# RchalYang/torchrl

Hardware: AMD Instinct MI355X
Metric: env_steps_per_sec_ppo_2048env_halfcheetah_shape (higher is better)
Workload: dtype f32

## Files before the change

torchrl_amd/csrc/k_rollout.hip:

```cpp
#include <algorithm>
#include "trl_common.h"
#include "trl_mlp.h"
#include "trl_head.h"
#include "trl_philox.h"

#define RO_THREADS 256
#define RO_ENVS 16
#ifdef TRL_EXP_CLK
#define CLK_DECL long long clk_prev = clock64(); float clk_acc[8] = {0, 0, 0, 0, 0, 0, 0, 0};
#define CLK(ph) { const long long c_ = clock64(); clk_acc[ph] += (float)(c_ - clk_prev); clk_prev = c_; }
#else
#define CLK_DECL
#define CLK(ph)
#endif
#define RO_NB 16

struct RolloutDev {
  const float *pf_params, *vf_params, *env_A, *env_B;
  float reward_scale; int horizon; int64_t env_seed_base;
  float* cur_obs; int32_t *t_env, *cur_step, *episode_idx; float* ep_return;
  const float* noise; int64_t noise_step0;
  float *obs, *next_obs, *acts, *values, *rewards, *terminals, *time_limits, *old_logp;
  int rows, top, N, n_steps, max_episode_frames; float discount;
  double* epoch_reward; int32_t* ep_count; float* ep_log; int ep_cap; int step0;
  int tanh_action, deterministic, store;
  double* norm_state; float* policy_obs; double* norm_ws; float norm_clip; int norm_update, norm_partial_reset;
  double* clear_hdr;
  float* boot;
  uint32_t* pub_dst; const uint32_t* pub_src; int64_t pub_words;
  const uint32_t* noise_flag; uint32_t noise_stamp;
  int D, A;
  int n_ro_wg; const f32x4* stg_src; unsigned long long* stg_dst; int64_t stg_n4;
  const uint32_t* stg_ready; uint32_t stg_job; uint32_t* stg_state; uint32_t* stg_ack;
  int64_t cat_seed, cat_env0;
};
#define RO_STAGERS 16

template <int CTRL> __device__ __forceinline__ double ro_dpp_f64(double v) {
  const unsigned long long u = __builtin_bit_cast(unsigned long long, v);
  const unsigned lo = (unsigned)__builtin_amdgcn_update_dpp(0, (int)(unsigned)(u & 0xFFFFFFFFull), CTRL, 0xF, 0xF, false);
  const unsigned hi = (unsigned)__builtin_amdgcn_update_dpp(0, (int)(unsigned)(u >> 32), CTRL, 0xF, 0xF, false);
  return __builtin_bit_cast(double, ((unsigned long long)hi << 32) | lo);
}
__device__ __forceinline__ double ro_row_sum16(double v) {
  v += ro_dpp_f64<0x128>(v);
  v += ro_dpp_f64<0x124>(v);
  v += ro_dpp_f64<0x122>(v);
  v += ro_dpp_f64<0x121>(v);
  return v;
}
#define NORM_SLOT 40

template <int D, int H, int A, int HC_ = 8> struct RoShape {
  static_assert(H == 64 && D > 16 && D <= 32 && A <= 8, "instantiated for 16 < D <= 32, H == 64, A <= 8");
  static_assert(HC_ == 8 || HC_ == 16, "the head exchange carries half or all of the 16-row head tile");
  static constexpr int HC = HC_;
  static constexpr int O_B1 = 0, O_B2 = H, O_B3 = 2 * H, O_LS = O_B3 + HC, O_H1 = O_LS + 8, O_HP = O_H1 + H * TL,
                       O_EPS = O_HP + 4 * HC * 16, LDS_FLOATS = O_EPS + RO_NB * 8 * 16;
};

__device__ __forceinline__ void stage_block(const f32x4* __restrict__ src, unsigned long long* __restrict__ dst, int64_t n4,
                                            int wg, int wgs, int threads, uint32_t* __restrict__ state, uint32_t stamp,
                                            uint32_t* __restrict__ host_ack) {
  const int64_t stride = (int64_t)wgs * threads;
  for (int64_t e = (int64_t)wg * threads + threadIdx.x; e < n4; e += 4 * stride) {
    f32x4 v[4];
#pragma unroll
    for (int q = 0; q < 4; ++q) if (e + q * stride < n4) v[q] = src[e + q * stride];
#pragma unroll
    for (int q = 0; q < 4; ++q)
      if (e + q * stride < n4) {
        const unsigned long long lo = ((unsigned long long)__float_as_uint(v[q][1]) << 32) | __float_as_uint(v[q][0]);
        const unsigned long long hi = ((unsigned long long)__float_as_uint(v[q][3]) << 32) | __float_as_uint(v[q][2]);
        __hip_atomic_store(dst + 2 * (e + q * stride), lo, __ATOMIC_RELAXED, __HIP_MEMORY_SCOPE_AGENT);
        __hip_atomic_store(dst + 2 * (e + q * stride) + 1, hi, __ATOMIC_RELAXED, __HIP_MEMORY_SCOPE_AGENT);
      }
  }
  asm volatile("s_waitcnt vmcnt(0)" ::: "memory");
  __syncthreads();
  if (threadIdx.x == 0) {
    const unsigned before = __hip_atomic_fetch_add(state + 1, 1u, __ATOMIC_RELAXED, __HIP_MEMORY_SCOPE_AGENT);
    if (before == (unsigned)wgs - 1) {
      __hip_atomic_store(state + 1, 0u, __ATOMIC_RELAXED, __HIP_MEMORY_SCOPE_AGENT);
      __hip_atomic_store(state, stamp, __ATOMIC_RELAXED, __HIP_MEMORY_SCOPE_AGENT);
      if (host_ack) __hip_atomic_store(host_ack, stamp, __ATOMIC_RELAXED, __HIP_MEMORY_SCOPE_SYSTEM);
    }
  }
}

template <int D, int H, int A, int ACT, bool NORM, bool RT = false, int HEAD = HEAD_GAUSS>
__global__ __launch_bounds__(RO_THREADS, 1) void rollout_kernel(RolloutDev a) {
  using S = RoShape<D, H, A, HEAD == HEAD_SD ? 16 : 8>;
  constexpr bool WIDE = D > 17, CAT = HEAD == HEAD_CAT, SD = HEAD == HEAD_SD;
  static_assert(!CAT || RT, "the categorical head exists as a runtime-dims instantiation only");
  static_assert(!SD || (RT && !NORM), "the state-dependent-std head exists as a runtime-dims instantiation only");
  static_assert(!WIDE || RT, "the wide tile exists as a runtime-dims instantiation only");
  static_assert(!(RT && NORM), "the cooperative (normalised) rollout is instantiated for the benchmark shape");
  const int Dr = RT ? a.D : D, Ar = RT ? a.A : A;
  const int HW = SD ? 2 * Ar : Ar;
  const int F_W1 = 0, F_B1 = H * Dr, F_W2 = F_B1 + H, F_B2 = F_W2 + H * H, F_W3 = F_B2 + H, F_B3 = F_W3 + HW * H,
            F_LS = F_B3 + HW;
  __shared__ __attribute__((aligned(16))) float lds[S::LDS_FLOATS];
  if (!NORM && (int)blockIdx.x >= a.n_ro_wg) {
    __shared__ int s_go;
    if (threadIdx.x == 0) {
      const unsigned long long t0 = wall_clock64();
      int go = 1;
      while (__hip_atomic_load(a.stg_ready, __ATOMIC_RELAXED, __HIP_MEMORY_SCOPE_SYSTEM) != a.stg_job) {
        __builtin_amdgcn_s_sleep(64);
        if (wall_clock64() - t0 > 3000ull) { go = 0; break; }
      }
      s_go = go;
    }
    __syncthreads();
    if (s_go)
      stage_block(a.stg_src, a.stg_dst, a.stg_n4, (int)blockIdx.x - a.n_ro_wg, (int)gridDim.x - a.n_ro_wg, RO_THREADS,
                  a.stg_state, a.stg_job, a.stg_ack);
    return;
  }
  const int tid = threadIdx.x, lane = tid & 63;
  const int mo = __builtin_amdgcn_readfirstlane(tid >> 6);
  const int j = lane & 15, g = lane >> 4, i = j;
  const int n = blockIdx.x * RO_ENVS + j;
  const bool valid = n < a.N;
  const float* gp = a.pf_params;
  const bool has_lo = g < Ar, has_hi = 4 + g < Ar;
  const int o_lo = has_lo ? g : 0, o_hi = has_hi ? 4 + g : 0;
  if (blockIdx.x == 0 && tid == 0 && a.clear_hdr) { a.clear_hdr[0] = 0.0; a.clear_hdr[1] = 0.0; }
  if (a.noise_flag && tid == 0) {
    unsigned spins = 0;
    while (__hip_atomic_load(a.noise_flag, __ATOMIC_RELAXED, __HIP_MEMORY_SCOPE_AGENT) != a.noise_stamp) {
      __builtin_amdgcn_s_sleep(32);
      if (++spins > (1u << 24)) {
        if (blockIdx.x == 0 && a.epoch_reward) a.epoch_reward[0] = __builtin_nan("");
        break;
      }
    }
    if (spins) __threadfence();
  }

  for (int e = tid; e < H; e += RO_THREADS) { lds[S::O_B1 + e] = gp[F_B1 + e]; lds[S::O_B2 + e] = gp[F_B2 + e]; }
  if constexpr (SD) {
    if (tid < 16) lds[S::O_B3 + tid] = tid < HW ? gp[F_B3 + (tid < HW ? tid : 0)] : 0.0f;
    if (tid < 8) lds[S::O_LS + tid] = 0.0f;
  } else if (tid < 8) {
    lds[S::O_B3 + tid] = tid < Ar ? gp[F_B3 + (tid < Ar ? tid : 0)] : 0.0f;
    lds[S::O_LS + tid] = (!CAT && tid < Ar) ? gp[F_LS + (tid < Ar ? tid : 0)] : 0.0f;
  }
  bool fv[4], fv2[4];
#pragma unroll
  for (int q = 0; q < 4; ++q) { fv[q] = 4 * g + q < Dr; fv2[q] = WIDE && 16 + 4 * g + q < Dr; }
  const bool f16 = !WIDE && 16 + g < Dr;
  const bool row_f = i < Dr, row_f2 = WIDE && 16 + i < Dr;
  constexpr int XK = WIDE ? 8 : 5, EK = XK + 2;
  float w1r[XK], w2r[4][4], w3a[4], we0[EK], w16[EK], we1[WIDE ? EK : 1];
  {
    const int row = 16 * mo + i;
#pragma unroll
    for (int r = 0; r < 4; ++r) w1r[r] = fv[r] ? gp[F_W1 + row * Dr + (fv[r] ? 4 * g + r : 0)] : 0.0f;
    if constexpr (WIDE) {
#pragma unroll
      for (int r = 0; r < 4; ++r) w1r[4 + r] = fv2[r] ? gp[F_W1 + row * Dr + (fv2[r] ? 16 + 4 * g + r : 0)] : 0.0f;
    } else {
      w1r[4] = f16 ? gp[F_W1 + row * Dr + (f16 ? 16 + g : 0)] : 0.0f;
    }
#pragma unroll
    for (int sl = 0; sl < 4; ++sl)
#pragma unroll
      for (int r = 0; r < 4; ++r) w2r[sl][r] = gp[F_W2 + row * H + 16 * sl + 4 * g + r];
#pragma unroll
    for (int r = 0; r < 4; ++r) w3a[r] = (i < HW) ? gp[F_W3 + (i < HW ? i : 0) * H + 16 * mo + 4 * g + r] : 0.0f;
    static_assert(WIDE || D == 17, "the narrow env step keeps exactly one feature outside the 16-row MFMA tile");
    const bool has16 = !WIDE && Dr > 16;
#pragma unroll
    for (int q = 0; q < EK; ++q) {
      const float* mat = q < XK ? a.env_A : a.env_B;
      int k; bool kin;
      if (q < 4) { k = 4 * g + q; kin = k < Dr; }
      else if (q < XK) { k = WIDE ? 16 + 4 * g + (q - 4) : 16 + g; kin = k < Dr; }
      else { k = (q == XK) ? g : 4 + g; kin = k < Ar; }
      const int kc = kin ? k : 0;
      we0[q] = (kin && row_f) ? mat[kc * Dr + (row_f ? i : 0)] : 0.0f;
      w16[q] = (kin && has16) ? mat[kc * Dr + (has16 ? 16 : 0)] : 0.0f;
      if constexpr (WIDE) we1[q] = (kin && row_f2) ? mat[kc * Dr + (row_f2 ? 16 + i : 0)] : 0.0f;
    }
  }
  __syncthreads();

  float* S_H1 = lds + S::O_H1;
  float* headp = lds + S::O_HP;
  float* S_EPS = lds + S::O_EPS;
  const float* b1s = lds + S::O_B1 + 16 * mo + 4 * g;
  const float* b2s = lds + S::O_B2 + 16 * mo + 4 * g;

  float ls_lo = fminf(fmaxf(lds[S::O_LS + o_lo], -20.0f), 2.0f), ls_hi = fminf(fmaxf(lds[S::O_LS + o_hi], -20.0f), 2.0f);
  float std_lo = __expf(ls_lo), std_hi = __expf(ls_hi);
  float iv_lo = __expf(-2.0f * ls_lo), iv_hi = __expf(-2.0f * ls_hi);
  const float b3_lo = lds[S::O_B3 + o_lo], b3_hi = lds[S::O_B3 + o_hi];

  float xb[XK];
#pragma unroll
  for (int r = 0; r < 4; ++r) xb[r] = (valid && fv[r]) ? a.cur_obs[(size_t)n * Dr + (fv[r] ? 4 * g + r : 0)] : 0.0f;
  if constexpr (WIDE) {
#pragma unroll
    for (int r = 0; r < 4; ++r) xb[4 + r] = (valid && fv2[r]) ? a.cur_obs[(size_t)n * Dr + (fv2[r] ? 16 + 4 * g + r : 0)] : 0.0f;
  } else {
    xb[4] = (valid && f16) ? a.cur_obs[(size_t)n * Dr + (f16 ? 16 + g : 0)] : 0.0f;
  }
  float xp[XK];
  __shared__ double s_mean[NORM ? D : 1], s_var[NORM ? D : 1], s_sum[NORM ? 2 * D + 1 : 1];
  __shared__ double s_cnt;
  unsigned* nhdr = NORM ? reinterpret_cast<unsigned*>(a.norm_ws) : nullptr;
  if constexpr (NORM) {
#pragma unroll
    for (int r = 0; r < 4; ++r) xp[r] = valid ? a.policy_obs[(size_t)n * D + 4 * g + r] : 0.0f;
    xp[4] = (valid && g == 0) ? a.policy_obs[(size_t)n * D + 16] : 0.0f;
    if (tid < D) { s_mean[tid] = a.norm_state[tid]; s_var[tid] = a.norm_state[D + tid]; }
    if (tid == 0) s_cnt = a.norm_state[2 * D];
    __syncthreads();
  } else {
#pragma unroll
    for (int q = 0; q < XK; ++q) xp[q] = xb[q];
  }
  int t_env = valid ? a.t_env[n] : 0;
  int cur_step = valid ? a.cur_step[n] : 0;
  int ep_idx = valid ? a.episode_idx[n] : 0;
  float ep_ret = valid ? a.ep_return[n] : 0.0f;
  const int64_t env_seed = a.env_seed_base + n;
  double rew_sum = 0.0;
  const bool dev_noise = !a.deterministic && !a.noise;
  CLK_DECL

  for (int t = 0; t < a.n_steps; ++t) {
    const int row = (a.top + t) % a.rows;
    const size_t cell = (size_t)row * a.N + n;

    float cat_u = 0.0f;
    if constexpr (CAT) {
      if (dev_noise && (t % RO_NB) == 0) {
        const int ts = 4 * mo + g;
        S_EPS[ts * 16 + j] = trl_cat_uniform(a.cat_seed, a.noise_step0 + t + ts, a.cat_env0 + n);
        __syncthreads();
      }
      if (dev_noise) cat_u = S_EPS[(t % RO_NB) * 16 + j];
    }
    if (!CAT && dev_noise && (t % RO_NB) == 0) {
      const int ts = 4 * mo + g;
      const int64_t gs = a.noise_step0 + t + ts;
      float z0[4], z1[4];
      philox_normals4((uint32_t)(gs & 0xFFFFFFFFll), (uint32_t)((gs >> 32) & 0xFFFFFFFFll), 0u, TRL_TAG_NOISE, env_seed, z0);
      if (Ar > 4)
        philox_normals4((uint32_t)(gs & 0xFFFFFFFFll), (uint32_t)((gs >> 32) & 0xFFFFFFFFll), 1u, TRL_TAG_NOISE, env_seed, z1);
#pragma unroll
      for (int c = 0; c < 4; ++c) {
        S_EPS[(ts * 8 + c) * 16 + j] = z0[c];
        if (4 + c < Ar) S_EPS[(ts * 8 + 4 + c) * 16 + j] = z1[c];
      }
      __syncthreads();
    }
    float eps_lo = 0.0f, eps_hi = 0.0f;
    if (!CAT && dev_noise) {
      eps_lo = S_EPS[((t % RO_NB) * 8 + o_lo) * 16 + j];
      eps_hi = S_EPS[((t % RO_NB) * 8 + o_hi) * 16 + j];
    } else if (!CAT && a.noise) {
      eps_lo = valid ? a.noise[((size_t)t * a.N + n) * Ar + o_lo] : 0.0f;
      eps_hi = valid ? a.noise[((size_t)t * a.N + n) * Ar + o_hi] : 0.0f;
    }

    CLK(0)
    f32x4 h1 = *reinterpret_cast<const f32x4*>(b1s);
#pragma unroll
    for (int q = 0; q < XK; ++q) h1 = mfma16(w1r[q], xp[q], h1);
    f32x4 e0 = f32x4{0.f, 0.f, 0.f, 0.f}, e1 = f32x4{0.f, 0.f, 0.f, 0.f};
    float p16 = 0.0f;
#pragma unroll
    for (int q = 0; q < XK; ++q) {
      e0 = mfma16(we0[q], xb[q], e0);
      if constexpr (WIDE) e1 = mfma16(we1[q], xb[q], e1);
      else p16 = fmaf(w16[q], xb[q], p16);
    }
#pragma unroll
    for (int r = 0; r < 4; ++r) h1[r] = act_fn<ACT>(h1[r]);
    store_T(S_H1, mo, h1, j, g);
    CLK(1)
    __syncthreads();
    CLK(2)
    f32x4 h2 = *reinterpret_cast<const f32x4*>(b2s), h2b = f32x4{0.f, 0.f, 0.f, 0.f};
#pragma unroll
    for (int sl = 0; sl < 4; sl += 2) {
      const f32x4 b0 = load_T(S_H1, sl, j, g), b1 = load_T(S_H1, sl + 1, j, g);
#pragma unroll
      for (int r = 0; r < 4; ++r) { h2 = mfma16(w2r[sl][r], b0[r], h2); h2b = mfma16(w2r[sl + 1][r], b1[r], h2b); }
    }
#pragma unroll
    for (int r = 0; r < 4; ++r) h2[r] = act_fn<ACT>(h2[r] + h2b[r]);
    f32x4 hp = f32x4{0.f, 0.f, 0.f, 0.f};
#pragma unroll
    for (int r = 0; r < 4; ++r) hp = mfma16(w3a[r], h2[r], hp);
    if (SD || g < 2) {
#pragma unroll
      for (int r = 0; r < 4; ++r) headp[(mo * S::HC + 4 * g + r) * 16 + j] = hp[r];
    }
    CLK(3)
    __syncthreads();
    CLK(4)
    float mean_lo = b3_lo, mean_hi = b3_hi;
#pragma unroll
    for (int w = 0; w < 4; ++w) { mean_lo += headp[(w * S::HC + o_lo) * 16 + j]; mean_hi += headp[(w * S::HC + o_hi) * 16 + j]; }
    if constexpr (SD) {
      float raw_lo = lds[S::O_B3 + Ar + o_lo], raw_hi = lds[S::O_B3 + Ar + o_hi];
#pragma unroll
      for (int w = 0; w < 4; ++w) {
        raw_lo += headp[(w * S::HC + Ar + o_lo) * 16 + j];
        raw_hi += headp[(w * S::HC + Ar + o_hi) * 16 + j];
      }
      ls_lo = fminf(fmaxf(raw_lo, -20.0f), 2.0f); ls_hi = fminf(fmaxf(raw_hi, -20.0f), 2.0f);
      std_lo = __expf(ls_lo); std_hi = __expf(ls_hi);
      iv_lo = __expf(-2.0f * ls_lo); iv_hi = __expf(-2.0f * ls_hi);
    }

    int cat_k = 0;
    float cat_lsel = 0.0f, cat_m = 0.0f, cat_S = 1.0f;
    if constexpr (CAT) {
      float lg[8], ex[8];
#pragma unroll
      for (int k = 0; k < 8; ++k) {
        float l = lds[S::O_B3 + k];
#pragma unroll
        for (int w = 0; w < 4; ++w) l += headp[(w * 8 + k) * 16 + j];
        lg[k] = l;
      }
      cat_m = lg[0];
#pragma unroll
      for (int k = 1; k < 8; ++k)
        if (k < Ar && lg[k] > cat_m) { cat_m = lg[k]; cat_k = k; }
      cat_S = 0.0f;
#pragma unroll
      for (int k = 0; k < 8; ++k)
        if (k < Ar) { ex[k] = expf(lg[k] - cat_m); cat_S += ex[k]; }
      if (dev_noise) {
        const float thr = cat_u * cat_S;
        float c = 0.0f;
        bool hit = false;
        cat_k = Ar - 1;
#pragma unroll
        for (int k = 0; k < 8; ++k)
          if (k < Ar) {
            c += ex[k];
            if (!hit && c >= thr) { cat_k = k; hit = true; }
          }
      }
#pragma unroll
      for (int k = 0; k < 8; ++k) cat_lsel = k == cat_k ? lg[k] : cat_lsel;
    }
    const float z_lo = fmaf(std_lo, eps_lo, mean_lo), z_hi = fmaf(std_hi, eps_hi, mean_hi);
    const float act_lo = CAT ? (g == cat_k ? 1.0f : 0.0f) : has_lo ? (a.tanh_action ? trl_tanh(z_lo) : z_lo) : 0.0f;
    const float act_hi = CAT ? (4 + g == cat_k ? 1.0f : 0.0f) : has_hi ? (a.tanh_action ? trl_tanh(z_hi) : z_hi) : 0.0f;
    e0 = mfma16(we0[XK], act_lo, e0);
    e0 = mfma16(we0[XK + 1], act_hi, e0);
    if constexpr (WIDE) {
      e1 = mfma16(we1[XK], act_lo, e1);
      e1 = mfma16(we1[XK + 1], act_hi, e1);
    } else {
      p16 = fmaf(w16[XK], act_lo, p16);
      p16 = fmaf(w16[XK + 1], act_hi, p16);
    }
    const f32x4 zero4 = f32x4{0.f, 0.f, 0.f, 0.f};
    const float e16 = WIDE ? 0.0f : mfma16(1.0f, p16, zero4)[0];
    const float act_sq = mfma16(1.0f, fmaf(act_lo, act_lo, act_hi * act_hi), zero4)[0];
    float logp = 0.0f;
    if (mo == 3) {
      if constexpr (CAT) {
        logp = (cat_lsel - cat_m) - logf(cat_S);
      } else {
        float zc, lp = 0.0f;
        if (has_lo) lp += gauss_logp_term(act_lo, mean_lo, iv_lo, ls_lo, a.tanh_action, zc);
        if (has_hi) lp += gauss_logp_term(act_hi, mean_hi, iv_hi, ls_hi, a.tanh_action, zc);
        logp = mfma16(1.0f, lp, zero4)[0];
      }
    }
    CLK(5)
    float nx[XK];
#pragma unroll
    for (int r = 0; r < 4; ++r) nx[r] = trl_tanh(e0[r]);
    if constexpr (WIDE) {
#pragma unroll
      for (int r = 0; r < 4; ++r) nx[4 + r] = trl_tanh(e1[r]);
    } else {
      nx[4] = (g == 0 && Dr > 16) ? trl_tanh(e16) : 0.0f;
    }

    CLK(6)
    const float nx0 = mfma16(1.0f, g == 0 ? nx[0] : 0.0f, zero4)[0];
    const float raw_rew = a.reward_scale * (nx0 - 0.1f * act_sq);
    t_env += 1; cur_step += 1;
    const bool done = t_env >= a.horizon;
    const bool surpass = cur_step >= a.max_episode_frames;
    float nxn[XK];
    bool any_reset = false;
    if constexpr (NORM) {
      if (a.norm_update) {
        double* part = a.norm_ws + 2 + (size_t)((t & 1) * gridDim.x + blockIdx.x) * NORM_SLOT;
        if (mo == 0) {
#pragma unroll
          for (int q = 0; q < 5; ++q) {
            const int f = q < 4 ? 4 * g + q : 16;
            const double d = (valid && (q < 4 || g == 0)) ? (double)nx[q] - s_mean[f] : 0.0;
            const double s1 = ro_row_sum16(d), s2 = ro_row_sum16(d * d);
            if (j == 0 && (q < 4 || g == 0)) {
              __hip_atomic_store(part + f, s1, __ATOMIC_RELAXED, __HIP_MEMORY_SCOPE_AGENT);
              __hip_atomic_store(part + D + f, s2, __ATOMIC_RELAXED, __HIP_MEMORY_SCOPE_AGENT);
            }
          }
          const bool fl = __ballot(valid && (done || surpass)) != 0ull;
          if (lane == 0) __hip_atomic_store(part + 2 * D, fl ? 1.0 : 0.0, __ATOMIC_RELAXED, __HIP_MEMORY_SCOPE_AGENT);
          asm volatile("s_waitcnt vmcnt(0)" ::: "memory");
          const unsigned long long stamp = (unsigned long long)(a.noise_step0 + t + 1);
          if (lane == 0)
            __hip_atomic_store(reinterpret_cast<unsigned long long*>(part + NORM_SLOT - 1), stamp, __ATOMIC_RELAXED,
                               __HIP_MEMORY_SCOPE_AGENT);
          for (int w = lane; w < (int)gridDim.x; w += 64) {
            const unsigned long long* st = reinterpret_cast<const unsigned long long*>(
                a.norm_ws + 2 + (size_t)((t & 1) * gridDim.x + w) * NORM_SLOT + NORM_SLOT - 1);
            int it = 0;
            while (__hip_atomic_load(st, __ATOMIC_RELAXED, __HIP_MEMORY_SCOPE_AGENT) != stamp) {
              __builtin_amdgcn_s_sleep(1);
              if (++it > (1 << 22)) { __hip_atomic_store(nhdr + 2, 1u, __ATOMIC_RELAXED, __HIP_MEMORY_SCOPE_AGENT); break; }
            }
          }
        }
        __syncthreads();
        if (tid < 2 * D + 1) {
          const double* col = a.norm_ws + 2 + (size_t)((t & 1) * gridDim.x) * NORM_SLOT + tid;
          double acc = 0.0;
          int w = 0;
          for (; w + 8 <= (int)gridDim.x; w += 8) {
            double v[8];
#pragma unroll
            for (int k = 0; k < 8; ++k) v[k] = __hip_atomic_load(col + (size_t)(w + k) * NORM_SLOT, __ATOMIC_RELAXED, __HIP_MEMORY_SCOPE_AGENT);
#pragma unroll
            for (int k = 0; k < 8; ++k) acc += v[k];
          }
          for (; w < (int)gridDim.x; ++w) acc += __hip_atomic_load(col + (size_t)w * NORM_SLOT, __ATOMIC_RELAXED, __HIP_MEMORY_SCOPE_AGENT);
          s_sum[tid] = acc;
        }
        __syncthreads();
        if (tid < D) {
          const double bn = (double)a.N, cnt = s_cnt;
          const double delta = s_sum[tid] / bn, bvar = fmax(s_sum[D + tid] / bn - delta * delta, 0.0);
          const double tot = cnt + bn;
          const double m2 = s_var[tid] * cnt + bvar * bn + delta * delta * cnt * bn / tot;
          s_mean[tid] += delta * bn / tot;
          s_var[tid] = m2 / tot;
        }
        __syncthreads();
        if (tid == 0) s_cnt += (double)a.N;
        any_reset = s_sum[2 * D] != 0.0;
      } else {
        any_reset = __ballot(valid && (done || surpass)) != 0ull;
      }
#pragma unroll
      for (int q = 0; q < 5; ++q) {
        const int f = q < 4 ? 4 * g + q : 16;
        const double z = ((double)nx[q] - s_mean[f]) / (sqrt(s_var[f]) + 1e-4);
        nxn[q] = (q < 4 || g == 0) ? (float)fmin(fmax(z, -(double)a.norm_clip), (double)a.norm_clip) : 0.0f;
      }
    } else {
#pragma unroll
      for (int q = 0; q < XK; ++q) nxn[q] = nx[q];
    }
    ep_ret += raw_rew;
    if (mo == 0 && g == 0 && valid) {
      rew_sum += (double)raw_rew;
      if (done) {
        const int slot = atomicAdd(a.ep_count, 1);
        if (slot < a.ep_cap) { a.ep_log[slot * 3 + 0] = (float)(a.step0 + t); a.ep_log[slot * 3 + 1] = (float)n; a.ep_log[slot * 3 + 2] = ep_ret; }
      }
    }
    if (done) ep_ret = 0.0f;

    float xn[XK];
#pragma unroll
    for (int q = 0; q < XK; ++q) xn[q] = nx[q];
    if (done || surpass) {
      ep_idx += 1; t_env = 0; cur_step = 0;
      float z[4];
      philox_normals4((uint32_t)ep_idx, 0u, (uint32_t)g, TRL_TAG_RESET, env_seed, z);
#pragma unroll
      for (int c = 0; c < 4; ++c) xn[c] = fv[c] ? z[c] : 0.0f;
      if constexpr (WIDE) {
        philox_normals4((uint32_t)ep_idx, 0u, (uint32_t)(4 + g), TRL_TAG_RESET, env_seed, z);
#pragma unroll
        for (int c = 0; c < 4; ++c) xn[4 + c] = fv2[c] ? z[c] : 0.0f;
      } else {
        xn[4] = 0.0f;
        if (g == 0 && Dr > 16) {
          philox_normals4((uint32_t)ep_idx, 0u, 4u, TRL_TAG_RESET, env_seed, z);
          xn[4] = z[0];
        }
      }
    }

    if (valid && a.store) {
      if (mo == 0 || mo == 1) {
        float* dst = (mo == 0 ? a.obs : a.next_obs) + cell * Dr;
        const float* src = mo == 0 ? xp : nxn;
#pragma unroll
        for (int r = 0; r < 4; ++r) if (!RT || fv[r]) dst[4 * g + r] = src[r];
        if constexpr (WIDE) {
#pragma unroll
          for (int r = 0; r < 4; ++r) if (fv2[r]) dst[16 + 4 * g + r] = src[4 + r];
        } else {
          if (g == 0 && (!RT || Dr > 16)) dst[16] = src[4];
        }
      } else if (mo == 2) {
        if constexpr (CAT) {
          if (g == 0) a.acts[cell] = (float)cat_k;
        } else {
          if (has_lo) a.acts[cell * Ar + g] = act_lo;
          if (has_hi) a.acts[cell * Ar + 4 + g] = act_hi;
        }
      } else {
        float* dst = g == 0 ? a.values : g == 1 ? a.rewards : g == 2 ? a.terminals : a.time_limits;
        const float val = g == 0 ? (surpass ? 1.0f : 0.0f) : g == 1 ? raw_rew
                        : g == 2 ? ((done || surpass) ? 1.0f : 0.0f) : (done ? 1.0f : 0.0f);
        dst[cell] = val;
        if (g == 0 && a.old_logp) a.old_logp[cell] = logp;
      }
    }
    if constexpr (NORM) {
#pragma unroll
      for (int q = 0; q < 5; ++q) {
        float alt = xn[q];
        if (a.norm_partial_reset) {
          const int f = q < 4 ? 4 * g + q : 16;
          const double z = ((double)xn[q] - s_mean[f]) / (sqrt(s_var[f]) + 1e-4);
          alt = (q < 4 || g == 0) ? (float)fmin(fmax(z, -(double)a.norm_clip), (double)a.norm_clip) : 0.0f;
        }
        xp[q] = any_reset ? alt : nxn[q];
      }
    } else {
#pragma unroll
      for (int q = 0; q < XK; ++q) xp[q] = xn[q];
    }
#pragma unroll
    for (int q = 0; q < XK; ++q) xb[q] = xn[q];
    CLK(7)
  }
  if constexpr (NORM) {
    if (mo == 0 && valid) {
#pragma unroll
      for (int r = 0; r < 4; ++r) a.policy_obs[(size_t)n * D + 4 * g + r] = xp[r];
      if (g == 0) a.policy_obs[(size_t)n * D + 16] = xp[4];
    }
    if (blockIdx.x == 0 && a.norm_update) {
      if (tid < D) { a.norm_state[tid] = s_mean[tid]; a.norm_state[D + tid] = s_var[tid]; }
      if (tid == 0) a.norm_state[2 * D] = s_cnt;
    }
  }
#ifdef TRL_EXP_CLK
  if (blockIdx.x == 0 && lane == 0)
    for (int ph = 0; ph < 8; ++ph) a.ep_log[(a.ep_cap - 16) * 3 + mo * 8 + ph] = clk_acc[ph];
#endif

  if (mo == 0 && valid) {
    float* dst = a.cur_obs + (size_t)n * Dr;
#pragma unroll
    for (int r = 0; r < 4; ++r) if (!RT || fv[r]) dst[4 * g + r] = xb[r];
    if constexpr (WIDE) {
#pragma unroll
      for (int r = 0; r < 4; ++r) if (fv2[r]) dst[16 + 4 * g + r] = xb[4 + r];
    }
    if (g == 0) {
      if (!WIDE && (!RT || Dr > 16)) dst[16] = xb[4];
      a.t_env[n] = t_env; a.cur_step[n] = cur_step; a.episode_idx[n] = ep_idx; a.ep_return[n] = ep_ret;
    }
  }
  if (mo == 0) {
    const double tot = wave_sum(rew_sum);
    if (lane == 0 && a.epoch_reward) atomicAdd(a.epoch_reward, tot);
  }
}

#define VP_THREADS 256

struct ValueDev {
  const float* vf_params; const float *obs, *next_obs; float *values, *rewards;
  int rows, top, N, n_steps; float discount;
  float* boot;
  uint32_t* pub_dst; const uint32_t* pub_src; int64_t pub_words;
  int D;
};

template <int D, int H, int ACT, bool RT = false>
__global__ __launch_bounds__(VP_THREADS, RT ? 1 : 2) void value_pass_kernel(ValueDev a) {
  static_assert(H == 64 && D > 16 && D <= 32, "instantiated for 16 < D <= 32, H == 64");
  constexpr bool WIDE = D > 17;
  static_assert(!WIDE || RT, "the wide tile exists as a runtime-dims instantiation only");
  constexpr int XK = WIDE ? 8 : 5;
  const int Dr = RT ? a.D : D;
  const int F_W1 = 0, F_B1 = H * Dr, F_W2 = F_B1 + H, F_B2 = F_W2 + H * H, F_W3 = F_B2 + H, F_B3 = F_W3 + H;
  __shared__ __attribute__((aligned(16))) float sb[2 * H];
  const int tid = threadIdx.x, lane = tid & 63, wave = tid >> 6;
  const int j = lane & 15, g = lane >> 4, i = j;
  const float* gp = a.vf_params;
  for (int e = tid; e < H; e += VP_THREADS) { sb[e] = gp[F_B1 + e]; sb[H + e] = gp[F_B2 + e]; }
  bool fv[4], fv2[4];
#pragma unroll
  for (int q = 0; q < 4; ++q) { fv[q] = 4 * g + q < Dr; fv2[q] = WIDE && 16 + 4 * g + q < Dr; }
  const bool f16 = !WIDE && 16 + g < Dr;
  const bool w2_al = !RT || ((reinterpret_cast<uintptr_t>(gp + F_W2) & 15) == 0);
  float w1[4][XK], w2[4][4][4], w3[4][4];
#pragma unroll
  for (int so = 0; so < 4; ++so) {
    const int row = 16 * so + i;
#pragma unroll
    for (int r = 0; r < 4; ++r) w1[so][r] = fv[r] ? gp[F_W1 + row * Dr + (fv[r] ? 4 * g + r : 0)] : 0.0f;
    if constexpr (WIDE) {
#pragma unroll
      for (int r = 0; r < 4; ++r) w1[so][4 + r] = fv2[r] ? gp[F_W1 + row * Dr + (fv2[r] ? 16 + 4 * g + r : 0)] : 0.0f;
    } else {
      w1[so][4] = f16 ? gp[F_W1 + row * Dr + (f16 ? 16 + g : 0)] : 0.0f;
    }
#pragma unroll
    for (int sl = 0; sl < 4; ++sl) {
      f32x4 w;
      if (w2_al) w = *reinterpret_cast<const f32x4*>(gp + F_W2 + row * H + 16 * sl + 4 * g);
      else __builtin_memcpy(&w, gp + F_W2 + row * H + 16 * sl + 4 * g, 16);
#pragma unroll
      for (int r = 0; r < 4; ++r) w2[so][sl][r] = w[r];
    }
#pragma unroll
    for (int r = 0; r < 4; ++r) w3[so][r] = gp[F_W3 + 16 * so + 4 * g + r];
  }
  const float b3 = gp[F_B3];
  __syncthreads();

  auto fetch = [&](const float* src, size_t cell, bool ok, float (&xb)[XK]) {
#pragma unroll
    for (int r = 0; r < 4; ++r) xb[r] = (ok && fv[r]) ? src[cell * Dr + (fv[r] ? 4 * g + r : 0)] : 0.0f;
    if constexpr (WIDE) {
#pragma unroll
      for (int r = 0; r < 4; ++r) xb[4 + r] = (ok && fv2[r]) ? src[cell * Dr + (fv2[r] ? 16 + 4 * g + r : 0)] : 0.0f;
    } else {
      xb[4] = (ok && f16) ? src[cell * Dr + (f16 ? 16 + g : 0)] : 0.0f;
    }
  };
  auto forward = [&](const float (&xb)[XK]) -> float {
    f32x4 h1[4], h2[4];
#pragma unroll
    for (int so = 0; so < 4; ++so) {
      f32x4 acc = *reinterpret_cast<const f32x4*>(sb + 16 * so + 4 * g);
#pragma unroll
      for (int q = 0; q < XK; ++q) acc = mfma16(w1[so][q], xb[q], acc);
#pragma unroll
      for (int r = 0; r < 4; ++r) acc[r] = act_fn<ACT>(acc[r]);
      h1[so] = acc;
    }
#pragma unroll
    for (int so = 0; so < 4; ++so) {
      f32x4 acc = *reinterpret_cast<const f32x4*>(sb + H + 16 * so + 4 * g);
#pragma unroll
      for (int sl = 0; sl < 4; ++sl)
#pragma unroll
        for (int r = 0; r < 4; ++r) acc = mfma16(w2[so][sl][r], h1[sl][r], acc);
#pragma unroll
      for (int r = 0; r < 4; ++r) acc[r] = act_fn<ACT>(acc[r]);
      h2[so] = acc;
    }
    float v = 0.0f;
#pragma unroll
    for (int so = 0; so < 4; ++so)
#pragma unroll
      for (int r = 0; r < 4; ++r) v = fmaf(w3[so][r], h2[so][r], v);
    v += __shfl_xor(v, 16, 64);
    v += __shfl_xor(v, 32, 64);
    return v + b3;
  };

  for (int64_t e = (int64_t)blockIdx.x * VP_THREADS + tid; e < a.pub_words; e += (int64_t)gridDim.x * VP_THREADS)
    a.pub_dst[e] = a.pub_src[e];
  const int64_t M = (int64_t)a.n_steps * a.N;
  const int64_t n_tiles = (M + 15) / 16;
  auto locate = [&](int64_t tile, bool& ok, int& t, int& n) -> size_t {
    const int64_t m = tile * 16 + j;
    ok = tile < n_tiles && m < M;
    t = ok ? (int)(m / a.N) : 0;
    n = ok ? (int)(m - (int64_t)t * a.N) : 0;
    return (size_t)((a.top + t) % a.rows) * a.N + n;
  };
  const int64_t stride = (int64_t)gridDim.x * 4;
  int64_t tile = (int64_t)blockIdx.x * 4 + wave;
  bool ok, ok_n;
  int t, n, t_n, n_n;
  float xb[XK], xn[XK];
  size_t cell = locate(tile, ok, t, n), cell_n;
  fetch(a.obs, cell, ok, xb);
  float marker = ok ? a.values[cell] : 0.0f, marker_n;
  for (; tile < n_tiles; tile += stride) {
    cell_n = locate(tile + stride, ok_n, t_n, n_n);
    fetch(a.obs, cell_n, ok_n, xn);
    marker_n = ok_n ? a.values[cell_n] : 0.0f;
    const float v = forward(xb);
    if (ok && g == 0) a.values[cell] = v;
    const bool last = ok && a.boot && t == a.n_steps - 1;
    if (__ballot(marker != 0.0f || last) != 0ull) {
      float x2[XK];
      fetch(a.next_obs, cell, ok, x2);
      const float v2 = forward(x2);
      if (ok && g == 0 && marker != 0.0f) a.rewards[cell] += a.discount * v2;
      if (last && g == 0) a.boot[n] = v2;
    }
#pragma unroll
    for (int q = 0; q < XK; ++q) xb[q] = xn[q];
    cell = cell_n; ok = ok_n; t = t_n; n = n_n; marker = marker_n;
  }
}

__global__ __launch_bounds__(256) void zero_value_pass_kernel(float* __restrict__ values, int rows, int top, int N, int n_steps,
                                                              float* __restrict__ boot, uint32_t* __restrict__ pub_dst,
                                                              const uint32_t* __restrict__ pub_src, int64_t pub_words) {
  const int64_t e0 = (int64_t)blockIdx.x * 256 + threadIdx.x, stride = (int64_t)gridDim.x * 256;
  for (int64_t e = e0; e < pub_words; e += stride) pub_dst[e] = pub_src[e];
  const int64_t M = (int64_t)n_steps * N;
  for (int64_t m = e0; m < M; m += stride) {
    const int t = (int)(m / N), n = (int)(m - (int64_t)t * N);
    values[(size_t)((top + t) % rows) * N + n] = 0.0f;
  }
  if (boot)
    for (int64_t n = e0; n < N; n += stride) boot[n] = 0.0f;
}

template <int D, int H, int A, int ACT>
static int rollout_norm_capacity() {
  int dev = 0, cus = 0, per_cu = 0;
  if (hipGetDevice(&dev) != hipSuccess) return 0;
  if (hipDeviceGetAttribute(&cus, hipDeviceAttributeMultiprocessorCount, dev) != hipSuccess) return 0;
  if (hipOccupancyMaxActiveBlocksPerMultiprocessor(&per_cu, rollout_kernel<D, H, A, ACT, true>, RO_THREADS, 0) != hipSuccess)
    return 0;
  return cus * per_cu * RO_ENVS;
}

template <int D, int H, int A, int ACT, bool RT = false, int HEAD = HEAD_GAUSS>
static int launch_rollout(const RolloutDev& d, hipStream_t s, hipEvent_t value_wait = nullptr) {
  const int n_wg = trl_ceil_div(d.N, RO_ENVS);
  if constexpr (RT) {
    if (d.norm_state) { trl_set_error("rollout: the normalised rollout is instantiated for the benchmark shape only"); return TRL_EUNSUPPORTED; }
    RolloutDev e = d;
    e.n_ro_wg = n_wg;
    hipLaunchKernelGGL((rollout_kernel<D, H, A, ACT, false, true, HEAD>), dim3(n_wg + (e.stg_n4 ? RO_STAGERS : 0)), dim3(RO_THREADS), 0, s, e);
  } else if (d.norm_state) {
    const int cap = rollout_norm_capacity<D, H, A, ACT>();
    if (d.norm_update && d.N > cap) {
      trl_set_error("rollout: %d envs with a running normaliser exceed the %d that can be co-resident", d.N, cap);
      return TRL_EUNSUPPORTED;
    }
    hipLaunchKernelGGL((rollout_kernel<D, H, A, ACT, true>), dim3(n_wg), dim3(RO_THREADS), 0, s, d);
  } else {
    RolloutDev e = d;
    e.n_ro_wg = n_wg;
    hipLaunchKernelGGL((rollout_kernel<D, H, A, ACT, false>), dim3(n_wg + (e.stg_n4 ? RO_STAGERS : 0)), dim3(RO_THREADS), 0, s, e);
  }
  TRL_LAUNCH_CHECK();
  if (d.store && !d.vf_params) {
    const int64_t blocks = ((int64_t)d.n_steps * d.N + 255) / 256;
    hipLaunchKernelGGL(zero_value_pass_kernel, dim3((unsigned)(blocks > 1024 ? 1024 : blocks)), dim3(256), 0, s, d.values, d.rows,
                       d.top, d.N, d.n_steps, d.boot, d.pub_dst, d.pub_src, d.pub_words);
    TRL_LAUNCH_CHECK();
  } else if (d.store) {
    if (value_wait) {
      hipError_t e = hipStreamWaitEvent(s, value_wait, 0);
      if (e != hipSuccess) { trl_set_error("rollout: hipStreamWaitEvent(value_wait_event): %s", hipGetErrorString(e)); return (int)e; }
    }
    ValueDev v{d.vf_params, d.obs, d.next_obs, d.values, d.rewards, d.rows, d.top, d.N, d.n_steps, d.discount, d.boot,
               d.pub_dst, d.pub_src, d.pub_words, d.D};
    const int64_t n_tiles = ((int64_t)d.n_steps * d.N + 15) / 16;
    const int grid = (int)(n_tiles / 4 + 1 < 512 ? n_tiles / 4 + 1 : 512);
    hipLaunchKernelGGL((value_pass_kernel<D, H, ACT, RT>), dim3(grid), dim3(VP_THREADS), 0, s, v);
    TRL_LAUNCH_CHECK();
  }
  return TRL_OK;
}

__global__ __launch_bounds__(256) void stage_h2d_kernel(const f32x4* __restrict__ src, unsigned long long* __restrict__ dst,
                                                        int64_t n4, uint32_t* __restrict__ state, uint32_t stamp) {
  stage_block(src, dst, n4, (int)blockIdx.x, (int)gridDim.x, 256, state, stamp, nullptr);
}
extern "C" int trl_stage_h2d_f32(const float* host_src, float* dev_dst, int64_t n, uint32_t* state, uint32_t stamp,
                                 void* stream) {
  TRL_REQUIRE(n >= 0 && (n & 3) == 0, "stage_h2d: n must be a multiple of 4");
  TRL_REQUIRE(state, "stage_h2d: null state");
  TRL_REQUIRE(!n || (host_src && dev_dst && ((reinterpret_cast<uintptr_t>(host_src) | reinterpret_cast<uintptr_t>(dev_dst)) & 15) == 0),
              "stage_h2d: null / misaligned pointer");
  const int grid = (int)std::max<int64_t>(1, std::min<int64_t>(16, (n / 4 + 1023) / 1024));
  hipLaunchKernelGGL(stage_h2d_kernel, dim3(grid), dim3(256), 0, (hipStream_t)stream, reinterpret_cast<const f32x4*>(host_src),
                     reinterpret_cast<unsigned long long*>(dev_dst), n / 4, state, stamp);
  TRL_LAUNCH_CHECK();
  return TRL_OK;
}

extern "C" int trl_rollout_supported(int D, int H, int A, int act) { return head_supported(HEAD_GAUSS, D, H, A, act); }
extern "C" int trl_rollout_cat_supported(int D, int H, int A, int act) { return head_supported(HEAD_CAT, D, H, A, act); }
extern "C" int trl_rollout_sd_supported(int D, int H, int A, int act) { return head_supported(HEAD_SD, D, H, A, act); }

static int rollout_synth(const trl_rollout_t* p, void* stream, int head, int64_t cat_seed = 0, int64_t cat_env0 = 0) {
  if (!p) { trl_set_error("rollout: null descriptor"); return TRL_EINVAL; }
  TRL_REQUIRE(p->pf_params && p->env_A && p->env_B, "null network / env pointer");
  TRL_REQUIRE(p->cur_obs && p->t_env && p->cur_step && p->episode_idx && p->ep_return, "null env state pointer");
  const bool all_ring = p->obs && p->next_obs && p->acts && p->values && p->rewards && p->terminals && p->time_limits;
  const bool no_ring = !p->obs && !p->next_obs && !p->acts && !p->values && !p->rewards && !p->terminals && !p->time_limits;
  TRL_REQUIRE(all_ring || no_ring, "ring tensors must be all set or all NULL");
  TRL_REQUIRE(p->ep_count && p->ep_log && p->ep_cap >= 0, "null episode log");
  TRL_REQUIRE(p->N > 0 && p->n_steps >= 0 && p->rows > 0, "bad sizes");
  TRL_REQUIRE(p->top >= 0 && p->top < p->rows, "top outside ring");
  TRL_REQUIRE(no_ring || p->n_steps <= p->rows, "n_steps exceeds ring rows");
  TRL_REQUIRE(p->horizon > 0 && p->max_episode_frames > 0, "horizon / max_episode_frames must be positive");
  if (head == HEAD_CAT) {
    TRL_REQUIRE(cat_env0 >= 0, "categorical: negative env offset");
    TRL_REQUIRE(!p->noise && !p->noise_flag && !p->stage_n,
                "categorical: actions are drawn from the device Philox stream only (no host noise block, nothing staged)");
    TRL_REQUIRE(!p->norm_state, "categorical: no running observation normaliser in the persistent rollout");
  }
  if (head == HEAD_SD) {
    TRL_REQUIRE(!p->norm_state, "state-dependent std: no running observation normaliser in the persistent rollout");
    TRL_REQUIRE(!p->noise_flag && !p->stage_n,
                "state-dependent std: the noise block is stream-ordered in front of the launch (no noise gate, nothing staged)");
  }
  if (head != HEAD_GAUSS && !head_supported(head, p->D, p->H, p->A, p->act)) {
    trl_set_error("rollout: %s shape D=%d H=%d A=%d act=%d not instantiated", HEADS[head].name, p->D, p->H, p->A, p->act);
    return TRL_EUNSUPPORTED;
  }
  if (p->n_steps == 0) return TRL_OK;
  RolloutDev d;
  d.pf_params = p->pf_params; d.vf_params = p->vf_params; d.env_A = p->env_A; d.env_B = p->env_B;
  d.reward_scale = p->reward_scale; d.horizon = p->horizon; d.env_seed_base = p->env_seed_base;
  d.cur_obs = p->cur_obs; d.t_env = p->t_env; d.cur_step = p->cur_step; d.episode_idx = p->episode_idx;
  d.ep_return = p->ep_return; d.noise = p->noise; d.noise_step0 = p->noise_step0;
  d.obs = p->obs; d.next_obs = p->next_obs; d.acts = p->acts; d.values = p->values; d.rewards = p->rewards;
  d.terminals = p->terminals; d.time_limits = p->time_limits; d.old_logp = p->old_logp;
  d.rows = p->rows; d.top = p->top; d.N = p->N; d.n_steps = p->n_steps;
  d.max_episode_frames = p->max_episode_frames; d.discount = p->discount;
  d.epoch_reward = p->epoch_reward; d.ep_count = p->ep_count; d.ep_log = p->ep_log; d.ep_cap = p->ep_cap;
  d.step0 = p->step0; d.tanh_action = p->tanh_action; d.deterministic = p->deterministic; d.store = all_ring ? 1 : 0;
  d.norm_state = p->norm_state; d.policy_obs = p->policy_obs; d.norm_ws = p->norm_workspace; d.norm_clip = p->norm_clip;
  d.norm_update = p->norm_update; d.norm_partial_reset = p->normalize_partial_reset;
  d.clear_hdr = p->clear_header; d.boot = all_ring ? p->boot_values : nullptr;
  TRL_REQUIRE(p->publish_words >= 0 && (!p->publish_words || (p->publish_dst && p->publish_src && all_ring)) &&
              ((reinterpret_cast<uintptr_t>(p->publish_dst) | reinterpret_cast<uintptr_t>(p->publish_src)) & 3) == 0,
              "publish: needs ring tensors, non-null 4-byte aligned pointers");
  d.pub_dst = (uint32_t*)p->publish_dst; d.pub_src = (const uint32_t*)p->publish_src; d.pub_words = p->publish_words;
// ... 236 lines not shown
```

Measured before the change: 102.8 million.

## Split Gaussian log-prob across waves and defer reduction to next step

Moves the per-step Gaussian log-prob terms off wave 3 onto waves 2 and 1, which write partial terms to a new LDS slot. Wave 3 reduces them during the next step's layer-2 phase and writes old_logp one step late, with a final flush after the loop. It also hoists the bias loads and replaces the per-step modulo row/cell index arithmetic with incrementing byte offsets for the stores and host-noise loads. The aim is to shorten the critical path of the slowest wave, at the cost of extra LDS traffic and a one-step-delayed write that relies on the existing barriers for ordering.

```diff
diff --git a/torchrl_amd/csrc/k_rollout.hip b/torchrl_amd/csrc/k_rollout.hip
--- a/torchrl_amd/csrc/k_rollout.hip
+++ b/torchrl_amd/csrc/k_rollout.hip
@@ -56,7 +56,7 @@
   static_assert(HC_ == 8 || HC_ == 16, "the head exchange carries half or all of the 16-row head tile");
   static constexpr int HC = HC_;
   static constexpr int O_B1 = 0, O_B2 = H, O_B3 = 2 * H, O_LS = O_B3 + HC, O_H1 = O_LS + 8, O_HP = O_H1 + H * TL,
-                       O_EPS = O_HP + 4 * HC * 16, LDS_FLOATS = O_EPS + RO_NB * 8 * 16;
+                       O_EPS = O_HP + 4 * HC * 16, O_LP = O_EPS + RO_NB * 8 * 16, LDS_FLOATS = O_LP + 2 * 64;
 };
 
 __device__ __forceinline__ void stage_block(const f32x4* __restrict__ src, unsigned long long* __restrict__ dst, int64_t n4,
@@ -229,12 +229,36 @@
   const int64_t env_seed = a.env_seed_base + n;
   double rew_sum = 0.0;
   const bool dev_noise = !a.deterministic && !a.noise;
+
+  const f32x4 b1v = *reinterpret_cast<const f32x4*>(b1s), b2v = *reinterpret_cast<const f32x4*>(b2s);
+  const int Wk = CAT ? 1 : Ar;
+  const int kst = mo < 2 ? Dr : mo == 2 ? Wk : 1;
+  char* const kbase = reinterpret_cast<char*>((mo == 0 ? a.obs : mo == 1 ? a.next_obs : a.acts) + (size_t)blockIdx.x * RO_ENVS * kst);
+  const size_t rpitch = (size_t)a.N * kst * sizeof(float);
+  int row = a.top;
+  size_t roff = (size_t)row * rpitch;
+  const unsigned o_x = (unsigned)(j * Dr + 4 * g) * 4u;
+  const unsigned o_a = (unsigned)(j * Wk + (CAT ? 0 : g)) * 4u;
+  char* const sbase = reinterpret_cast<char*>((g == 0 ? a.values : g == 1 ? a.rewards : g == 2 ? a.terminals : a.time_limits)
+                                              + (valid ? n : 0));
+  char* const lbase = reinterpret_cast<char*>(a.old_logp + (size_t)blockIdx.x * RO_ENVS);
+  const unsigned o_l = (unsigned)j * 4u;
+  const bool want_lp = a.store && a.old_logp;
+  const bool host_noise = !CAT && !dev_noise && a.noise;
+  const float* nzp = a.noise + (size_t)blockIdx.x * RO_ENVS * Ar;
+  const size_t npitch = (size_t)a.N * Ar;
+  const unsigned o_nlo = (unsigned)((valid ? j : 0) * Ar + o_lo) * 4u, o_nhi = (unsigned)((valid ? j : 0) * Ar + o_hi) * 4u;
+  auto ldb = [](const float* base, unsigned byte_off) -> float {
+    return *reinterpret_cast<const float*>(reinterpret_cast<const char*>(base) + byte_off);
+  };
+  constexpr bool LP_SPLIT = !CAT;
+  constexpr int RO_W_LO = 2, RO_W_HI = 1;
+  float* const S_LP = lds + S::O_LP;
+  size_t roff_prev = 0;
+  float lp_a = 0.0f, lp_b = 0.0f, logp_prev = 0.0f;
   CLK_DECL
 
   for (int t = 0; t < a.n_steps; ++t) {
-    const int row = (a.top + t) % a.rows;
-    const size_t cell = (size_t)row * a.N + n;
-
     float cat_u = 0.0f;
     if constexpr (CAT) {
       if (dev_noise && (t % RO_NB) == 0) {
@@ -262,13 +286,14 @@
     if (!CAT && dev_noise) {
       eps_lo = S_EPS[((t % RO_NB) * 8 + o_lo) * 16 + j];
       eps_hi = S_EPS[((t % RO_NB) * 8 + o_hi) * 16 + j];
-    } else if (!CAT && a.noise) {
-      eps_lo = valid ? a.noise[((size_t)t * a.N + n) * Ar + o_lo] : 0.0f;
-      eps_hi = valid ? a.noise[((size_t)t * a.N + n) * Ar + o_hi] : 0.0f;
+    } else if (host_noise) {
+      eps_lo = valid ? ldb(nzp, o_nlo) : 0.0f;
+      eps_hi = valid ? ldb(nzp, o_nhi) : 0.0f;
+      nzp += npitch;
     }
 
     CLK(0)
-    f32x4 h1 = *reinterpret_cast<const f32x4*>(b1s);
+    f32x4 h1 = b1v;
 #pragma unroll
     for (int q = 0; q < XK; ++q) h1 = mfma16(w1r[q], xp[q], h1);
     f32x4 e0 = f32x4{0.f, 0.f, 0.f, 0.f}, e1 = f32x4{0.f, 0.f, 0.f, 0.f};
@@ -285,7 +310,9 @@
     CLK(1)
     __syncthreads();
     CLK(2)
-    f32x4 h2 = *reinterpret_cast<const f32x4*>(b2s), h2b = f32x4{0.f, 0.f, 0.f, 0.f};
+    f32x4 h2 = b2v, h2b = f32x4{0.f, 0.f, 0.f, 0.f};
+    const bool lp_due = LP_SPLIT && mo == 3 && want_lp && t > 0;
+    if (lp_due) { lp_a = S_LP[lane]; lp_b = S_LP[64 + lane]; }
 #pragma unroll
     for (int sl = 0; sl < 4; sl += 2) {
       const f32x4 b0 = load_T(S_H1, sl, j, g), b1 = load_T(S_H1, sl + 1, j, g);
@@ -300,6 +327,12 @@
     if (SD || g < 2) {
 #pragma unroll
       for (int r = 0; r < 4; ++r) headp[(mo * S::HC + 4 * g + r) * 16 + j] = hp[r];
+    }
+    if (lp_due) {
+      float lp = 0.0f;
+      lp += lp_a;
+      lp += lp_b;
+      logp_prev = mfma16(1.0f, lp, f32x4{0.f, 0.f, 0.f, 0.f})[0];
     }
     CLK(3)
     __syncthreads();
@@ -369,15 +402,17 @@
     const float e16 = WIDE ? 0.0f : mfma16(1.0f, p16, zero4)[0];
     const float act_sq = mfma16(1.0f, fmaf(act_lo, act_lo, act_hi * act_hi), zero4)[0];
     float logp = 0.0f;
-    if (mo == 3) {
-      if constexpr (CAT) {
-        logp = (cat_lsel - cat_m) - logf(cat_S);
-      } else {
-        float zc, lp = 0.0f;
-        if (has_lo) lp += gauss_logp_term(act_lo, mean_lo, iv_lo, ls_lo, a.tanh_action, zc);
-        if (has_hi) lp += gauss_logp_term(act_hi, mean_hi, iv_hi, ls_hi, a.tanh_action, zc);
-        logp = mfma16(1.0f, lp, zero4)[0];
-      }
+    if constexpr (LP_SPLIT) {
+      if (want_lp && mo == RO_W_LO) {
+        float zc;
+        S_LP[lane] = has_lo ? gauss_logp_term(act_lo, mean_lo, iv_lo, ls_lo, a.tanh_action, zc) : 0.0f;
+      }
+      if (want_lp && mo == RO_W_HI) {
+        float zc;
+        S_LP[64 + lane] = has_hi ? gauss_logp_term(act_hi, mean_hi, iv_hi, ls_hi, a.tanh_action, zc) : 0.0f;
+      }
+    } else if (mo == 3) {
+      logp = (cat_lsel - cat_m) - logf(cat_S);
     }
     CLK(5)
     float nx[XK];
@@ -503,31 +538,38 @@
 
     if (valid && a.store) {
       if (mo == 0 || mo == 1) {
-        float* dst = (mo == 0 ? a.obs : a.next_obs) + cell * Dr;
+        float* dst = reinterpret_cast<float*>(kbase + roff + o_x);
         const float* src = mo == 0 ? xp : nxn;
 #pragma unroll
-        for (int r = 0; r < 4; ++r) if (!RT || fv[r]) dst[4 * g + r] = src[r];
+        for (int r = 0; r < 4; ++r) if (!RT || fv[r]) dst[r] = src[r];
         if constexpr (WIDE) {
 #pragma unroll
-          for (int r = 0; r < 4; ++r) if (fv2[r]) dst[16 + 4 * g + r] = src[4 + r];
+          for (int r = 0; r < 4; ++r) if (fv2[r]) dst[16 + r] = src[4 + r];
         } else {
           if (g == 0 && (!RT || Dr > 16)) dst[16] = src[4];
         }
       } else if (mo == 2) {
+        float* dst = reinterpret_cast<float*>(kbase + roff + o_a);
         if constexpr (CAT) {
-          if (g == 0) a.acts[cell] = (float)cat_k;
+          if (g == 0) dst[0] = (float)cat_k;
         } else {
-          if (has_lo) a.acts[cell * Ar + g] = act_lo;
-          if (has_hi) a.acts[cell * Ar + 4 + g] = act_hi;
+          if (has_lo) dst[0] = act_lo;
+          if (has_hi) dst[4] = act_hi;
         }
       } else {
-        float* dst = g == 0 ? a.values : g == 1 ? a.rewards : g == 2 ? a.terminals : a.time_limits;
         const float val = g == 0 ? (surpass ? 1.0f : 0.0f) : g == 1 ? raw_rew
                         : g == 2 ? ((done || surpass) ? 1.0f : 0.0f) : (done ? 1.0f : 0.0f);
-        dst[cell] = val;
-        if (g == 0 && a.old_logp) a.old_logp[cell] = logp;
-      }
-    }
+        *reinterpret_cast<float*>(sbase + roff) = val;
+        if constexpr (LP_SPLIT) {
+          if (g == 0 && lp_due) *reinterpret_cast<float*>(lbase + roff_prev + o_l) = logp_prev;
+        } else {
+          if (g == 0 && a.old_logp) *reinterpret_cast<float*>(lbase + roff + o_l) = logp;
+        }
+      }
+    }
+    roff_prev = roff;
+    roff += rpitch;
+    if (++row == a.rows) { row = 0; roff = 0; }
     if constexpr (NORM) {
 #pragma unroll
       for (int q = 0; q < 5; ++q) {
@@ -546,6 +588,18 @@
 #pragma unroll
     for (int q = 0; q < XK; ++q) xb[q] = xn[q];
     CLK(7)
+  }
+  if constexpr (LP_SPLIT) {
+    if (want_lp && a.n_steps > 0) {
+      __syncthreads();
+      if (mo == 3) {
+        float lp = 0.0f;
+        lp += S_LP[lane];
+        lp += S_LP[64 + lane];
+        const float last = mfma16(1.0f, lp, f32x4{0.f, 0.f, 0.f, 0.f})[0];
+        if (valid && g == 0) *reinterpret_cast<float*>(lbase + roff_prev + o_l) = last;
+      }
+    }
   }
   if constexpr (NORM) {
     if (mo == 0 && valid) {
```

New measurement: 103.3 million (median of 6 runs). Within noise of the previous version (+0.5%).
